# IDEA-Research/SegDINO3D

Hardware: AMD Instinct MI355X
Metric: scenes/sec forward (ScanNet200 ~150k pts, 200 queries) (higher is better)
Workload: dtype f32; 1 GPU; configs[1]: ScanNet-val-like scenes; a STEP is one scene; `value` times the K scenes as 28 evaluation forwards of 4/5 scenes each (`forward_sizes`), 4 forward(s) in flight per GPU (<= 20 scenes in flight); `single_scene` = one forward of one scene in flight; fp32 sparse backbone (Res16UNet34C) + fp32 decoder + post-processing, device-resident in/out; points=150000, superpoints=3000, queries_2d=300, scene_layout=benchmark, query_num=200, parallelism=scene-sharded x1, streams=4, max_scenes_per_forward=5, scenes_in_flight_per_gpu=20, gpu_numa_node=-1

## Files before the change

### include/segdino3d_hip.h

```cpp
#ifndef SEGDINO3D_HIP_H
#define SEGDINO3D_HIP_H

#include <stddef.h>
#include <stdint.h>

#ifdef __cplusplus
extern "C" {
#endif

#define SD3D_ABI_VERSION 2

int sd3d_abi_version(void);
const char* sd3d_last_error(void);
int sd3d_selftest_host(void);
int sd3d_set_scenes_in_flight(int n);

int sd3d_set_pair_pool(int on);
int sd3d_pair_pool_check(void);
int sd3d_pair_pool_launches(int64_t* launches_out);
int sd3d_pair_pool_poison(int64_t word);

size_t sd3d_sort_ws_bytes(int64_t n);
int sd3d_sort_pairs_u64_ex(uint64_t* keys_in, uint32_t* vals_in, uint64_t* keys_out, uint32_t* vals_out, uint32_t* vals_scratch,
                           int64_t n, int begin_bit, int end_bit, void* ws, size_t ws_bytes, int* landed_in_input, void* stream);
size_t sd3d_scan_ws_bytes(int64_t n);
int sd3d_scan_exclusive_i32(const int32_t* in, int32_t* out, int64_t n, int32_t* total_dev, void* ws, size_t ws_bytes,
                            void* stream);
int sd3d_keys_from_f32(const float* x, int64_t n, int descending, uint64_t* keys, void* stream);
int sd3d_keys_from_i64(const int64_t* x, int64_t n, uint64_t* keys, void* stream);
int sd3d_keys_from_i64_checked(const int64_t* x, int64_t n, uint64_t* keys, int bits, int32_t* flag, int flag_value, void* stream);
int sd3d_keys_from_i64_checked_max(const int64_t* x, int64_t n, uint64_t* keys, int bits, int32_t* flag, int flag_value, int32_t* max_out,
                                   void* stream);

int sd3d_keys_from_i64_offset_checked_max(const int64_t* x, int64_t n, int64_t add, uint64_t* keys, int bits, int32_t* flag, int flag_value,
                                          int32_t* max_out, void* stream);

size_t sd3d_scene_stats_ws_bytes(void);
int sd3d_scene_stats(const float* points, int ld, int64_t n, float* stats, void* ws, size_t ws_bytes, void* stream);
int sd3d_voxel_keys(const float* points, int ld, int64_t n, float inv_voxel, const float* stats, int shift_to_min,
                    int batch_index, int32_t* origin, uint64_t* keys, int32_t* icoords, int32_t* err_flag, void* stream);
size_t sd3d_unique_ws_bytes(int64_t n_cap);
int sd3d_unique_sorted(const uint64_t* keys, const uint32_t* src_idx, int64_t n_cap, const int32_t* n_dev, int shift,
                       uint64_t* ukeys, int32_t* seg_start, int32_t* map, int32_t* n_unique_dev, void* ws,
                       size_t ws_bytes, const float* clip_stats, float clip_inv_voxel, int clip_level, int clip_min_shape,
                       void* stream);
size_t sd3d_unique_levels_ws_bytes(int64_t n_cap, int n_extra);
int sd3d_unique_levels(const uint64_t* keys, int64_t n_cap, const int32_t* n_dev, int n_extra, uint64_t* const* ukeys,
                       int32_t* const* parents, int32_t* counts, void* ws, size_t ws_bytes, void* stream);
typedef struct sd3d_voxelise_desc {
    const float* points; int64_t n; int ld; int shift_to_min; float inv_voxel; int key_bits; int n_levels; int sp_bits;
// ... 375 lines not shown
```

### segdino3d_amd/_lib.py

```python
from __future__ import annotations

import ctypes as C
import os

_HERE = os.path.dirname(os.path.abspath(__file__))
LIB_PATH = os.environ.get("SD3D_LIB") or os.path.join(_HERE, "libsegdino3d_hip.so")
ABI_VERSION = 2

_lib = None

_p = C.c_void_p
_i = C.c_int
_l = C.c_int64
_z = C.c_size_t
_f = C.c_float

SIGNATURES = {
    "sd3d_abi_version": (_i, []),
    "sd3d_last_error": (C.c_char_p, []),
    "sd3d_set_scenes_in_flight": (_i, [_i]),
    "sd3d_set_pair_pool": (_i, [_i]),
    "sd3d_pair_pool_check": (_i, []),
    "sd3d_pair_pool_launches": (_i, [_p]),
    "sd3d_pair_pool_poison": (_i, [_l]),
    "sd3d_selftest_host": (_i, []),
    "sd3d_sort_ws_bytes": (_z, [_l]),
    "sd3d_sort_pairs_u64_ex": (_i, [_p, _p, _p, _p, _p, _l, _i, _i, _p, _z, _p, _p]),
    "sd3d_scan_ws_bytes": (_z, [_l]),
    "sd3d_scan_exclusive_i32": (_i, [_p, _p, _l, _p, _p, _z, _p]),
    "sd3d_keys_from_f32": (_i, [_p, _l, _i, _p, _p]),
    "sd3d_keys_from_i64": (_i, [_p, _l, _p, _p]),
    "sd3d_keys_from_i64_checked": (_i, [_p, _l, _p, _i, _p, _i, _p]),
    "sd3d_keys_from_i64_checked_max": (_i, [_p, _l, _p, _i, _p, _i, _p, _p]),
    "sd3d_keys_from_i64_offset_checked_max": (_i, [_p, _l, _l, _p, _i, _p, _i, _p, _p]),
    "sd3d_voxel_levels_all": (_i, [_p, _p, _l, _i, _p, _p, _p, _p, _p, _p, _z, _p]),
    "sd3d_voxelise_scene_ws_bytes": (_z, [_l, _i]),
    "sd3d_voxelise_scene": (_i, [_p, _p, _p]),
    "sd3d_scene_stats_ws_bytes": (_z, []),
    "sd3d_scene_stats": (_i, [_p, _i, _l, _p, _p, _z, _p]),
    "sd3d_voxel_keys": (_i, [_p, _i, _l, _f, _p, _i, _i, _p, _p, _p, _p, _p]),
    "sd3d_unique_ws_bytes": (_z, [_l]),
    "sd3d_unique_levels_ws_bytes": (_z, [_l, _i]),
    "sd3d_unique_levels": (_i, [_p, _l, _p, _i, _p, _p, _p, _p, _z, _p]),
    "sd3d_unique_sorted": (_i, [_p, _p, _l, _p, _i, _p, _p, _p, _p, _p, _z, _p, _f, _i, _i, _p]),
    "sd3d_hash_build": (_i, [_p, _l, _p, _p, _l, _p]),
    "sd3d_kernel_map": (_i, [_p, _l, _p, _p, _l, _p, _i, _i, _p, _p, _p]),
    "sd3d_kernel_maps_hier_ws_bytes": (_z, [_i, _p]),
    "sd3d_kernel_maps_hier": (_i, [_i, _p, _p, _p, _p, _p, _p, _p, _p, _p, _p, _p, _p, _p, _z, _p]),
    "sd3d_stride_maps": (_i, [_p, _p, _l, _l, _p, _p, _p, _p]),
    "sd3d_voxel_mean": (_i, [_p, _i, _p, _i, _i, _p, _l, _p, _p, _l, _p, _i, _p]),
    "sd3d_segment_starts": (_i, [_p, _l, _l, _p, _p]),
    "sd3d_voxel_mean_batch": (_i, [_p, _i, _i, _i, _p, _p, _p, _l, _p, _i, _p]),
    "sd3d_keys_from_i64_offset": (_i, [_p, _l, _l, _p, _p]),
    "sd3d_segment_starts_batch": (_i, [_p, _l, _l, _p, _i, _p, _p]),
# ... 140 lines not shown
```

### segdino3d_amd/csrc/pair_conv.h

```cpp
#pragma once
#include "common.h"
#include "../../include/segdino3d_hip.h"

#define PT 128
#define PG_CHAIN 0x40000000
#define PG_KMASK 0x3FFFFFFF

struct GGParams;

int launch_pair_conv(const float* in0, int ld0, int C0, const float* in1, int ld1, const int32_t* in_idx, const int32_t* tile_k,
                     int64_t p_cap, const int32_t* pos, const int32_t* rlist, int rl_stride, int center, const int32_t* out_idx,
                     const float* wt, int K, int Cin, int Cout, int64_t M, const float* scale,
                     const float* shift, const float* res, int ld_res, float* out, int ld_out, int act, float* part,
                     size_t part_bytes, hipStream_t st);
int launch_pair_dense(const GGParams& q, hipStream_t st);
```

### segdino3d_amd/csrc/pair_gemm.hip

```cpp
#include "gg_common.h"
#include "pair_conv.h"
#include <stdlib.h>
#include <atomic>
#include <vector>

static std::atomic<int> g_scenes_in_flight{1};
extern "C" int sd3d_set_scenes_in_flight(int n) { return g_scenes_in_flight.exchange(n < 1 ? 1 : n); }

#define PART_STORE4(PTR, V) do { if (p.nt_part) __builtin_nontemporal_store((V), (f32x4*)(PTR)); else *(f32x4*)(PTR) = (V); } while (0)
#define PART_LOAD4(PTR) __builtin_nontemporal_load((const f32x4*)(PTR))
#define PBS_LD 36

struct PGParams {
    const float* in0; int ld0; int C0;
    const float* in1; int ld1;
    const int32_t* in_idx;
    const int32_t* tile_k;
    const float* wt;
    int Cin, Cout;
    float* part;
    int n_tiles;
    const int32_t* out_idx;
    const float* scale; const float* shift; const float* res; int ld_res;
    float* out; int ld_out; int act;
// ... 15 lines not shown
    (void)__hip_atomic_fetch_max(ctr, (unsigned long long)epoch << 32, __ATOMIC_RELAXED, __HIP_MEMORY_SCOPE_AGENT);
}
__device__ __forceinline__ unsigned int pool_draw(unsigned long long* ctr, unsigned int epoch) {
    const unsigned long long old = __hip_atomic_fetch_add(ctr, 1ull, __ATOMIC_RELAXED, __HIP_MEMORY_SCOPE_AGENT);
    return (unsigned int)(old >> 32) == epoch ? (unsigned int)old : POOL_POISONED;
}
__global__ __launch_bounds__(256) void pool_check_kernel(unsigned long long tickets) {
    const int s = blockIdx.x * 256 + threadIdx.x;
    if (s >= PG_POOL_SLOTS) return;
    const unsigned long long last = tickets > (unsigned long long)s ? (tickets - 1 - s) / PG_POOL_SLOTS + 1 : 0;
    int bad = 0;
#pragma unroll
    for (int w = 0; w < PG_POOL_WORDS; ++w) {
        const unsigned long long v = g_pool_ctr[(size_t)s * PG_POOL_WORDS + w];
        if ((v >> 32) > last || ((v >> 32) == 0 && v != 0)) ++bad;
    }
    if (bad) atomicAdd(&g_pool_bad, (unsigned int)bad);
}


__device__ __forceinline__ float pg_affine(float x, const float* scale, const float* shift, int n) {
    return __builtin_fmaf(x, scale ? scale[n] : 1.f, shift ? shift[n] : 0.f);
}
__device__ __attribute__((noinline)) float pg_act_slow(float t, int act) {
    return act == 2 ? 0.5f * t * (1.f + erff(t * 0.70710678118654752440f)) : 1.f / (1.f + expf(-t));
}
__device__ __forceinline__ float pg_act(float t, int act) {
    if (act == 1) t = fmaxf(t, 0.f);
    else if (act >= 2) t = pg_act_slow(t, act);
    return t;
}

#define PG_PIECE 24
template <int NT, int MODE>
__device__ __forceinline__ void pair_gemm_body(const PGParams& p, float (*Bs)[NT * 32 * PBS_LD], int* Ix, int* Kx) {
    constexpr bool DIRECT = MODE >= 1;
    const int tid = threadIdx.x, lane = tid & 63;
    const int wv = __builtin_amdgcn_readfirstlane(tid >> 6);
    const int j = lane & 31, h = lane >> 5;
    constexpr bool dense = MODE == 2;
    const int n_real = dense ? (int)((p.dense_rows + PT - 1) / PT) : p.tile_k[p.n_tiles];
    const int nchunks = p.Cin >> 5;
    const bool pool = p.pool_ctr != nullptr && nchunks >= 3 && n_real >= 6 * (int)gridDim.x;
    int n_static = n_real;
    const int unit = (6 + nchunks - 1) / nchunks;
    if (pool) {
        if (tid == 0) pool_claim(p.pool_ctr + blockIdx.y, p.pool_epoch);
        n_static = (int)((int64_t)n_real * 13 / 16);
        if (p.chained) while (n_static < n_real && (p.tile_k[n_static - 1] & PG_CHAIN)) ++n_static;
    }
    int range0 = (int)((int64_t)blockIdx.x * n_static / gridDim.x);
    int range1 = (int)((int64_t)(blockIdx.x + 1) * n_static / gridDim.x);
    if (p.chained) {
        while (range0 > 0 && range0 < n_static && (p.tile_k[range0 - 1] & PG_CHAIN)) ++range0;
        while (range1 > 0 && range1 < n_static && (p.tile_k[range1 - 1] & PG_CHAIN)) ++range1;
    }
    if (range1 <= range0 && !pool) return;
    const int ncol0 = blockIdx.y * NT * 32;
    __shared__ int pool_unit;
    bool poisoned = false;
    int fallback_round = 0;
    const uint64_t wstride_b = (uint64_t)p.Cout * (uint64_t)p.Cin * 4ull;

    f32x16 acc[NT];
    const f32x16 zero16 = {0.f, 0.f, 0.f, 0.f, 0.f, 0.f, 0.f, 0.f, 0.f, 0.f, 0.f, 0.f, 0.f, 0.f, 0.f, 0.f};
    bool fresh = true;

    f32x4 bst[NT];
    uint32_t woff[NT];
#pragma unroll
    for (int i = 0; i < NT; ++i) {
        const int f = tid + i * 256;
        int n = ncol0 + (f >> 3);
        n = n < p.Cout ? n : p.Cout - 1;
        woff[i] = (uint32_t)(n * p.Cin + (f & 7) * 4) * 4u;
    }
    float* const sts = &Bs[0][(tid >> 3) * PBS_LD + (tid & 7) * 4];
    auto stage_load = [&](int kf, int chunk) {
        const int kw = p.k_flip >= 0 ? p.k_flip - (kf & PG_KMASK) : (kf & PG_KMASK);
        const char* Wk = (const char*)p.wt + (uint64_t)(uint32_t)kw * wstride_b + (uint32_t)chunk * 128u;
#pragma unroll
        for (int i = 0; i < NT; ++i) bst[i] = *(const f32x4*)(Wk + woff[i]);
    };
    auto stage_store = [&](int buf) {
#pragma unroll
        for (int i = 0; i < NT; ++i) *(f32x4*)(sts + buf * (NT * 32 * PBS_LD) + i * 32 * PBS_LD) = bst[i];
    };
    const uint64_t lane_b = (uint64_t)(h * 64);
    auto load_a = [&](f32x4 (&a)[4], int row, int chunk) {
        const int cc = chunk * 32;
        const bool first = cc < p.C0;
        const char* base = (const char*)(first ? p.in0 : p.in1) + (uint32_t)(first ? cc : cc - p.C0) * 4u;
        const uint32_t ld4 = (uint32_t)(first ? p.ld0 : p.ld1) * 4u;
        const char* src = base + ((uint64_t)(uint32_t)row * ld4 + lane_b);
#pragma unroll
        for (int q = 0; q < 4; ++q) a[q] = *(const f32x4*)(src + q * 16);
    };
    const bool full_cols = ncol0 + NT * 32 <= p.Cout;

  for (;;) {
    for (int piece0 = range0; piece0 < range1; piece0 += PG_PIECE) {
        const int ntl = range1 - piece0 < PG_PIECE ? range1 - piece0 : PG_PIECE;
        __syncthreads();
        if (dense) {
            for (int f = tid; f < ntl * PT; f += 256) {
                const int64_t r = (int64_t)piece0 * PT + f;
                Ix[f] = (int)(r < p.dense_rows ? r : p.dense_rows - 1);
            }
            if (tid < PG_PIECE + 2) Kx[tid] = 0;
        } else {
        for (int f = tid; f < ntl * PT; f += 256) {
            const int v = p.in_idx[(int64_t)piece0 * PT + f];
            Ix[f] = v < 0 ? 0 : v;
        }
        if (tid < PG_PIECE + 2) Kx[tid] = tid < ntl ? p.tile_k[piece0 + tid] : 0;
        }
        __syncthreads();
        const int nsteps = ntl * nchunks;
        const int* Iw = Ix + wv * 32 + j;
        int k_cur = __builtin_amdgcn_readfirstlane(Kx[0]), k_nxt = __builtin_amdgcn_readfirstlane(Kx[1]);
        f32x4 a0[4], a1[4], a2[4];
        int pf_t = 0, pf_c = 0;
#define PF_ADVANCE() do { if (++pf_c == nchunks) { pf_c = 0; ++pf_t; } } while (0)
#define PF_ROW() Iw[(pf_t < ntl ? pf_t : ntl - 1) * PT]
        load_a(a0, PF_ROW(), pf_c); PF_ADVANCE();
        load_a(a1, PF_ROW(), pf_c); PF_ADVANCE();
        stage_load(k_cur, 0);
        stage_store(0);
        __syncthreads();
        int buf = 0, cur_lt = 0, cur_c = 0, s = 0;
#define PAIR_STEP(CUR, PF)                                                                                            \
    {                                                                                                                 \
        const bool has_next = s + 1 < nsteps;                                                                         \
        const bool last_chunk = cur_c + 1 == nchunks;                                                                 \
        const int pf_row = PF_ROW();                 \
        const int k_after = Kx[cur_lt + 2];                                                                           \
        {                                                                                                             \
            const float* bb = &Bs[buf][j * PBS_LD + h * 16];                                                          \
            f32x4 bq[2][NT];                                                                                          \
            _Pragma("unroll") for (int t = 0; t < NT; ++t) bq[0][t] = *(const f32x4*)(bb + t * 32 * PBS_LD);          \
            _Pragma("unroll") for (int q = 0; q < 4; ++q) {                                                           \
                if (q < 3) {                                                                                          \
                    _Pragma("unroll") for (int t = 0; t < NT; ++t)                                                    \
                        bq[(q + 1) & 1][t] = *(const f32x4*)(bb + t * 32 * PBS_LD + (q + 1) * 4);                     \
                }                                                                                                     \
                _Pragma("unroll") for (int e = 0; e < 4; ++e) {                                                       \
                    if (q == 0 && e == 0) {                                                                           \
                        if (fresh) {                                                                                  \
// ... 37 lines not shown
                _Pragma("unroll") for (int t = 0; t < NT; ++t)                                                        \
                    _Pragma("unroll") for (int g = 0; g < 4; ++g)                                                     \
                        if (full_cols || ncol0 + 4 * h + t * 32 + 8 * g < p.Cout)                                     \
                            PART_STORE4(dst + t * 32 + 8 * g, (f32x4{acc[t][4 * g], acc[t][4 * g + 1],                \
                                                                     acc[t][4 * g + 2], acc[t][4 * g + 3]}));         \
            }                                                                                                         \
            fresh = true;                                                                                             \
        } else {                                                                                                      \
            fresh = false;                                                                                            \
        }                                                                                                             \
        if (!has_next) break;                                                                                         \
        stage_store(buf ^ 1);                                                                                         \
        __syncthreads();                                                                                              \
        buf ^= 1;                                                                                                     \
        ++s;                                                                                                          \
        if (last_chunk) {                                                                                             \
            cur_c = 0; ++cur_lt;                                                                                      \
            k_cur = k_nxt; k_nxt = __builtin_amdgcn_readfirstlane(k_after);                                           \
        } else {                                                                                                      \
            ++cur_c;                                                                                                  \
        }                                                                                                             \
    }
        for (;;) {
            PAIR_STEP(a0, a2)
            PAIR_STEP(a1, a0)
            PAIR_STEP(a2, a1)
        }
#undef PAIR_STEP
#undef PF_ADVANCE
#undef PF_ROW
    }
    if (!pool) break;
    __syncthreads();
    if (tid == 0) {
        unsigned int d = poisoned ? POOL_POISONED : pool_draw(p.pool_ctr + blockIdx.y, p.pool_epoch);
        if (d == POOL_POISONED) {
            if (!poisoned) atomicAdd(&g_pool_bad_seen, 1u);
            d = blockIdx.x + (unsigned)fallback_round * gridDim.x;
            pool_unit = -1 - (int)d;
        } else {
            pool_unit = (int)d;
        }
    }
    __syncthreads();
    int u = __builtin_amdgcn_readfirstlane(pool_unit);
    if (u < 0) { poisoned = true; ++fallback_round; u = -1 - u; }
    range0 = n_static + u * unit;
    if (range0 >= n_real) break;
    range1 = range0 + unit < n_real ? range0 + unit : n_real;
    if (p.chained) {
        while (range0 < n_real && (p.tile_k[range0 - 1] & PG_CHAIN)) ++range0;
        while (range1 < n_real && (p.tile_k[range1 - 1] & PG_CHAIN)) ++range1;
    }
  }
}

#define PAIR_GEMM_ENTRY(NAME, NT, WAVES, MODE)                                                                  \
    __global__ __launch_bounds__(256) __attribute__((amdgpu_waves_per_eu(WAVES, WAVES))) void NAME(const PGParams p) { \
        __shared__ __attribute__((aligned(16))) float Bs[2][NT * 32 * PBS_LD];                                  \
        __shared__ int Ix[PG_PIECE * PT];                                                                       \
        __shared__ int Kx[PG_PIECE + 2];                                                                        \
        pair_gemm_body<NT, MODE>(p, Bs, Ix, Kx);                                                               \
    }
PAIR_GEMM_ENTRY(pair_gemm_kernel_1, 1, 3, 0)
PAIR_GEMM_ENTRY(pair_gemm_kernel_2, 2, 2, 0)
PAIR_GEMM_ENTRY(pair_gemm_kernel_3, 3, 2, 0)
PAIR_GEMM_ENTRY(pair_gemm_kernel_4, 4, 2, 0)
PAIR_GEMM_ENTRY(pair_gemm_direct_kernel_1, 1, 3, 1)
PAIR_GEMM_ENTRY(pair_gemm_direct_kernel_2, 2, 2, 1)
PAIR_GEMM_ENTRY(pair_gemm_direct_kernel_3, 3, 2, 1)
PAIR_GEMM_ENTRY(pair_gemm_direct_kernel_4, 4, 2, 1)
PAIR_GEMM_ENTRY(pair_dense_kernel_1, 1, 3, 2)
PAIR_GEMM_ENTRY(pair_dense_kernel_2, 2, 2, 2)
PAIR_GEMM_ENTRY(pair_dense_kernel_3, 3, 2, 2)
PAIR_GEMM_ENTRY(pair_dense_kernel_4, 4, 2, 2)

#define WS_RANGE_TILES 24
#define WS_STAGE_BATCH 16

#define LOAD_A4(A, PTR)                                                                                            \
    do { _Pragma("unroll") for (int q_ = 0; q_ < 4; ++q_) A[q_] = *(const f32x4*)((PTR) + q_ * 4); } while (0)

template <int NT, int RT, int ST, bool DIRECT>
__device__ __forceinline__ void pair_gemm_ws_body(const PGParams& p, float* Ws) {
    constexpr int UPT = 4 / RT;
    const int tid = threadIdx.x, lane = tid & 63;
    const int wv = __builtin_amdgcn_readfirstlane(tid >> 6);
    const int j = lane & 31, h = lane >> 5;
    const int n_real = p.tile_k[p.n_tiles];
    const int range0 = (int)((int64_t)blockIdx.x * n_real / gridDim.x);
    const int range1 = (int)((int64_t)(blockIdx.x + 1) * n_real / gridDim.x);
    if (range1 <= range0) return;
    const int nchunks = p.Cin >> 5;
    const int ldw = p.Cin + 4;
    const int c4 = p.Cin >> 2;
    const int npieces = 32 * NT * c4;
    const int ncol0 = blockIdx.y * NT * 32;
    int* Ix = (int*)(Ws + 32 * NT * ldw);

    f32x16 acc[RT][NT];
    const f32x16 zero16 = {0.f, 0.f, 0.f, 0.f, 0.f, 0.f, 0.f, 0.f, 0.f, 0.f, 0.f, 0.f, 0.f, 0.f, 0.f, 0.f};
    bool fresh = true;

  for (int tile0 = range0; tile0 < range1; tile0 += WS_RANGE_TILES) {
    const int ntl = range1 - tile0 < WS_RANGE_TILES ? range1 - tile0 : WS_RANGE_TILES;
    __syncthreads();
    for (int f = tid; f < ntl * PT; f += 256) {
        const int v = p.in_idx[(int64_t)(tile0 + (f >> 7)) * PT + (f & (PT - 1))];
// ... 271 lines not shown
    if (hipDeviceSynchronize() != hipSuccess) { sd3d_set_error(SD3D_ERR_LAUNCH, "pair_pool_check: device synchronisation failed"); return -1; }
    unsigned int zero = 0, bad = 0, seen = 0;
    if (hipMemcpyToSymbol(HIP_SYMBOL(g_pool_bad), &zero, sizeof(zero)) != hipSuccess) { sd3d_set_error(SD3D_ERR_LAUNCH, "pair_pool_check: symbol write failed"); return -1; }
    hipLaunchKernelGGL(pool_check_kernel, dim3(PG_POOL_SLOTS / 256), dim3(256), 0, nullptr, g_pool_tickets[dev].load(std::memory_order_relaxed));
    if (hipGetLastError() != hipSuccess || hipDeviceSynchronize() != hipSuccess ||
        hipMemcpyFromSymbol(&bad, HIP_SYMBOL(g_pool_bad), sizeof(bad)) != hipSuccess ||
        hipMemcpyFromSymbol(&seen, HIP_SYMBOL(g_pool_bad_seen), sizeof(seen)) != hipSuccess ||
        hipMemcpyToSymbol(HIP_SYMBOL(g_pool_bad_seen), &zero, sizeof(zero)) != hipSuccess) { sd3d_set_error(SD3D_ERR_LAUNCH, "pair_pool_check: check kernel failed"); return -1; }
    if (seen) sd3d_set_error(SD3D_ERR_LAUNCH, "pair_pool_check: launches met counter words no launch can have written (they fell back to a static split of their shared tail: results unaffected)");
    bad += seen;
    return (int)bad;
}
extern "C" int sd3d_pair_pool_launches(int64_t* launches_out) {
    int dev = 0;
    if (!launches_out || hipGetDevice(&dev) != hipSuccess || dev < 0 || dev >= PG_MAX_DEVICES) return sd3d_set_error(SD3D_ERR_ARG, "pair_pool_launches: no device / no output");
    *launches_out = (int64_t)g_pool_tickets[dev].load(std::memory_order_relaxed);
    return SD3D_OK;
}
extern "C" int sd3d_pair_pool_poison(int64_t word) {
    unsigned long long* base = nullptr;
    if (hipGetSymbolAddress((void**)&base, HIP_SYMBOL(g_pool_ctr)) != hipSuccess) return sd3d_set_error(SD3D_ERR_LAUNCH, "pair_pool_poison: no symbol");
    std::vector<unsigned long long> h((size_t)PG_POOL_SLOTS * PG_POOL_WORDS, (unsigned long long)word);
    if (hipDeviceSynchronize() != hipSuccess || hipMemcpy(base, h.data(), h.size() * sizeof(unsigned long long), hipMemcpyHostToDevice) != hipSuccess)
        return sd3d_set_error(SD3D_ERR_LAUNCH, "pair_pool_poison: copy failed");
    return SD3D_OK;
}

typedef void (*PGKernel)(const PGParams);
static const PGKernel k_lockstep[2][4] = {{pair_gemm_kernel_1, pair_gemm_kernel_2, pair_gemm_kernel_3, pair_gemm_kernel_4},
                                          {pair_gemm_direct_kernel_1, pair_gemm_direct_kernel_2, pair_gemm_direct_kernel_3, pair_gemm_direct_kernel_4}};
static const PGKernel k_ws[2][4] = {{pair_gemm_ws_kernel_1, pair_gemm_ws_kernel_2, pair_gemm_ws_kernel_3, pair_gemm_ws_kernel_4},
                                    {pair_gemm_ws_direct_kernel_1, pair_gemm_ws_direct_kernel_2, pair_gemm_ws_direct_kernel_3, pair_gemm_ws_direct_kernel_4}};
static const PGKernel k_dense[4] = {pair_dense_kernel_1, pair_dense_kernel_2, pair_dense_kernel_3, pair_dense_kernel_4};

static std::atomic<int> g_n_cu[PG_MAX_DEVICES];
static std::atomic<bool> g_ws_attr[PG_MAX_DEVICES];

static int pg_device(int* n_cu) {
    int dev = 0;
    if (hipGetDevice(&dev) != hipSuccess || dev < 0 || dev >= PG_MAX_DEVICES) return -1;
    int n = g_n_cu[dev].load(std::memory_order_relaxed);
    if (!n) {
        if (hipDeviceGetAttribute(&n, hipDeviceAttributeMultiprocessorCount, dev) != hipSuccess || n <= 0) return -1;
        g_n_cu[dev].store(n, std::memory_order_relaxed);
    }
    *n_cu = n;
    return dev;
}

static void pg_col_tiles(int Cout, int* nt_out, int* cgs_out) {
    const int sub = (Cout + 31) / 32;
    int nt = sub >= 4 ? 4 : sub;
    if (sub > 4 && sub % 4) { for (int c = 4; c >= 1; --c) if (sub % c == 0) { nt = c; break; } }
    *nt_out = nt;
    *cgs_out = (int)cdiv(sub, nt);
}

static dim3 pg_lockstep_grid(int n_cu, int nt, int cgs, int64_t tiles) {
    int gx = n_cu * (nt == 1 ? 3 : 2) / cgs;
    gx = gx < 1 ? 1 : (gx < tiles ? gx : (int)tiles);
    return dim3((unsigned)gx, (unsigned)cgs);
}

static void pg_setup_pool(PGParams& g, int dev, int cgs, hipStream_t st) {
    if (!pool_enabled() || cgs > PG_POOL_WORDS) return;
    hipStreamCaptureStatus cap = hipStreamCaptureStatusNone;
    if (st != nullptr && (hipStreamIsCapturing(st, &cap) != hipSuccess || cap != hipStreamCaptureStatusNone)) return;
    unsigned long long* base = g_pool_bases[dev].load(std::memory_order_acquire);
    if (!base && hipGetSymbolAddress((void**)&base, HIP_SYMBOL(g_pool_ctr)) == hipSuccess) g_pool_bases[dev].store(base, std::memory_order_release);
    if (!base) return;
    const unsigned long long t = g_pool_tickets[dev].fetch_add(1, std::memory_order_relaxed);
    g.pool_ctr = base + (size_t)(t % PG_POOL_SLOTS) * PG_POOL_WORDS;
    g.pool_epoch = (unsigned int)(t / PG_POOL_SLOTS + 1);
}

int launch_pair_conv(const float* in0, int ld0, int C0, const float* in1, int ld1, const int32_t* in_idx, const int32_t* tile_k,
                     int64_t p_cap, const int32_t* pos, const int32_t* rlist, int rl_stride, int center, const int32_t* out_idx,
                     const float* wt, int K, int Cin, int Cout, int64_t M, const float* scale,
                     const float* shift, const float* res, int ld_res, float* out, int ld_out, int act, float* part,
                     size_t part_bytes, hipStream_t st) {
    if (M <= 0 || Cout <= 0) return SD3D_OK;
    if (Cin <= 0 || (Cin & 31)) return sd3d_set_error(SD3D_ERR_ARG, "pair_conv: Cin must be a positive multiple of 32");
    if (Cout & 3) return sd3d_set_error(SD3D_ERR_ARG, "pair_conv: Cout must be a multiple of 4");
    if (in1 && ((C0 & 31) || C0 > Cin)) return sd3d_set_error(SD3D_ERR_ARG, "pair_conv: concat split must be a multiple of 32");
    if (!in1) C0 = Cin;
    if ((ld0 & 3) || (in1 && (ld1 & 3)) || (ld_out & 3)) return sd3d_set_error(SD3D_ERR_ARG, "pair_conv: row strides must be multiples of 4 floats");
    if (p_cap <= 0 || (p_cap % PT)) return sd3d_set_error(SD3D_ERR_ARG, "pair_conv: p_cap must be a positive multiple of 128");
    if (part_bytes < (size_t)p_cap * Cout * sizeof(float)) return sd3d_set_error(SD3D_ERR_ARG, "pair_conv: partial-product buffer too small");
    int n_cu = 0;
    const int dev = pg_device(&n_cu);
    if (dev < 0) return sd3d_set_error(SD3D_ERR_LAUNCH, "pair_conv: no device");
    if ((ld_res & 3) && res) return sd3d_set_error(SD3D_ERR_ARG, "pair_conv: residual row stride must be a multiple of 4 floats");
    const bool mirror_w = center == SD3D_PAIR_MIRROR_W(-1) || center == SD3D_PAIR_MIRROR_W(SD3D_PAIR_CHAINED);
    if (mirror_w) center += 2;
    if (center >= 0 || center < SD3D_PAIR_CHAINED) return sd3d_set_error(SD3D_ERR_ARG, "pair_conv: center must be -1 or SD3D_PAIR_CHAINED, or SD3D_PAIR_MIRROR_W of them (the dense centre kernel of round 3 left the library: profiles/EXPERIMENTS.md)");
    const bool direct = out_idx != nullptr;
    if (!direct && !rlist && !pos)
        return sd3d_set_error(SD3D_ERR_ARG, "pair_conv: pass 2 needs rlist, or pos, or out_idx (direct epilogue); "
                                            "this table was built without a position table (lean evaluation lists)");
    const bool crowded = g_scenes_in_flight.load(std::memory_order_relaxed) > 1;
    PGParams g;
    g.in0 = in0; g.ld0 = ld0; g.C0 = C0; g.in1 = in1; g.ld1 = ld1; g.in_idx = in_idx; g.tile_k = tile_k; g.wt = wt;
    g.Cin = Cin; g.Cout = Cout; g.part = part;
    g.chained = center == SD3D_PAIR_CHAINED ? 1 : 0;
    g.nt_part = crowded ? 1 : 0;
    g.dense_rows = 0;
    g.pool_ctr = nullptr;
    g.pool_epoch = 0;
    g.k_flip = mirror_w ? K - 1 : -1;
    g.out_idx = out_idx;
    g.scale = scale; g.shift = shift; g.res = res; g.ld_res = ld_res; g.out = out; g.ld_out = ld_out; g.act = act;
    int nt, cgs;
    pg_col_tiles(Cout, &nt, &cgs);
    g.n_tiles = (int)(p_cap / PT);
    const size_t w_lds = (size_t)Cout * (Cin + 4) * sizeof(float);
    const size_t w_lds_cg = (size_t)(32 * nt) * (Cin + 4) * sizeof(float);
    const bool ws_one = !g.chained && !(crowded && nt >= 3) && cgs == 1 && Cout == 32 * nt && w_lds <= 68 * 1024;
    const bool ws_two = !g.chained && !crowded && cgs == 2 && nt == 4 && Cout == 256 && g.n_tiles >= 1024 && w_lds_cg + WS_RANGE_TILES * PT * sizeof(int32_t) + 256 <= 160 * 1024;
    if (ws_one || ws_two) {
        if (!g_ws_attr[dev].load(std::memory_order_relaxed)) {
            for (int d = 0; d < 2; ++d)
                for (int i = 0; i < 4; ++i)
                    (void)hipFuncSetAttribute((const void*)k_ws[d][i], hipFuncAttributeMaxDynamicSharedMemorySize, (i == 3 ? 160 : 80) * 1024);
            g_ws_attr[dev].store(true, std::memory_order_relaxed);
        }
        int per_cu = nt == 1 ? 4 : (nt == 3 ? 3 : 2);
        const size_t w_need = ws_two ? w_lds_cg : w_lds;
        const int by_lds = (int)((160 * 1024) / (w_need + WS_RANGE_TILES * PT * sizeof(int32_t) + 256));
        per_cu = per_cu < by_lds ? per_cu : by_lds;
        int gx = n_cu * per_cu / (ws_two ? 2 : 1);
        gx = gx < 1 ? 1 : (gx < g.n_tiles ? gx : g.n_tiles);
        const size_t lds = w_need + (size_t)WS_RANGE_TILES * PT * sizeof(int32_t);
        hipLaunchKernelGGL(k_ws[direct][nt - 1], dim3((unsigned)gx, ws_two ? 2u : 1u), dim3(256), lds, st, g);
    } else {
        pg_setup_pool(g, dev, cgs, st);
        hipLaunchKernelGGL(k_lockstep[direct][nt - 1], pg_lockstep_grid(n_cu, nt, cgs, g.n_tiles), dim3(256), 0, st, g);
    }
    if (direct) {
    } else if (rlist) {
        PRLParams r;
        r.rlist = rlist; r.rl_stride = rl_stride; r.M = M; r.part = part; r.Cout = Cout; r.scale = scale; r.shift = shift; r.res = res;
        r.ld_res = ld_res; r.out = out; r.ld_out = ld_out; r.act = act;
        hipLaunchKernelGGL(pair_reduce_rl_kernel, dim3((unsigned)cdiv(M * (Cout / 4), 256)), dim3(256), 0, st, r);
    } else {
        PRParams r;
        r.pos = pos; r.K = K; r.M = M; r.part = part; r.Cout = Cout; r.scale = scale; r.shift = shift; r.res = res; r.ld_res = ld_res;
        r.out = out; r.ld_out = ld_out; r.act = act;
        hipLaunchKernelGGL(pair_reduce_kernel, dim3((unsigned)cdiv(M * (Cout / 4), 256)), dim3(256), 0, st, r);
    }
    SD3D_CHECK_LAUNCH();
    return SD3D_OK;
}
extern "C" int sd3d_pair_conv_ex(const float* in0, int ld0, int C0, const float* in1, int ld1, const int32_t* in_idx, const int32_t* tile_k,
                                 int64_t p_cap, const int32_t* pos, const int32_t* rlist, int rl_stride, int center, const int32_t* out_idx,
                                 const float* wt, int K, int Cin, int Cout, int64_t M, const float* scale, const float* shift, const float* res,
                                 int ld_res, float* out, int ld_out, int act, float* part, size_t part_bytes, void* stream) {
    return launch_pair_conv(in0, ld0, C0, in1, ld1, in_idx, tile_k, p_cap, pos, rlist, rl_stride, center, out_idx, wt, K, Cin, Cout, M,
                            scale, shift, res, ld_res, out, ld_out, act, part, part_bytes, (hipStream_t)stream);
}

int launch_pair_dense(const GGParams& q, hipStream_t st) {
    int n_cu = 0;
    if (pg_device(&n_cu) < 0) return sd3d_set_error(SD3D_ERR_LAUNCH, "pair_dense: no device");
    PGParams g;
    g.in0 = q.in0; g.ld0 = q.ld0; g.C0 = q.in1 ? q.C0 : q.Cin; g.in1 = q.in1; g.ld1 = q.ld1; g.in_idx = nullptr; g.tile_k = nullptr; g.wt = q.wt;
    g.Cin = q.Cin; g.Cout = q.Cout; g.part = nullptr; g.n_tiles = 0; g.out_idx = nullptr; g.scale = q.scale; g.shift = q.shift; g.res = q.res;
    g.ld_res = q.ld_res; g.out = q.out; g.ld_out = q.ld_out; g.act = q.act; g.nt_part = 0; g.chained = 0; g.dense_rows = q.M; g.pool_ctr = nullptr; g.pool_epoch = 0; g.k_flip = -1;
    int nt, cgs;
    pg_col_tiles(q.Cout, &nt, &cgs);
// ... 5 lines not shown
```

### segdino3d_amd/csrc/pair_lists.hip

```cpp
#include "pair_conv.h"

#define PL_ROWS 2048

__device__ static inline int block_excl_scan_256p(int v, int* total, int* smem4) {
    const int lane = threadIdx.x & 63, w = threadIdx.x >> 6;
    int inc = v;
#pragma unroll
    for (int d = 1; d < 64; d <<= 1) {
        int t = __shfl_up(inc, d);
        if (lane >= d) inc += t;
    }
    if (lane == 63) smem4[w] = inc;
    __syncthreads();
    int base = 0;
    for (int i = 0; i < w; ++i) base += smem4[i];
    *total = smem4[0] + smem4[1] + smem4[2] + smem4[3];
    __syncthreads();
    return base + inc - v;
}

#define PL_MAX_TABLES 16
#define RL_ROWS 256
struct PLTable {
    const int32_t* nbr; int32_t* pos; int32_t* in_idx; int32_t* tile_k; int32_t* blk_cnt; int32_t* totals;
// ... 356 lines not shown
    __syncthreads();
    for (int sg = tid; sg < nseg; sg += 256) {
        int run = T.blk_cnt[(int64_t)sg * T.nblk + blk];
#pragma unroll
        for (int w = 0; w < 4; ++w) { const int c = wb[w][sg]; wb[w][sg] = run; run += c; }
    }
    __syncthreads();
    for (int sg = blk; sg < nseg; sg += T.nblk) {
        const int g = sg / CH_NPAT, q = sg - g * CH_NPAT;
        const int ns = g == T.G ? 1 : ch_nsrc(q), nt = (seg_tot[sg] + PT - 1) / PT;
        for (int e = tid; e < nt * ns; e += 256) {
            const int sub = e % ns;
            int k;
            if (g == T.G) k = centre;
            else if (q == 0) k = g;
            else if (q == 1) k = T.K - 1 - g;
            else if (q == 2) k = sub == 0 ? g : T.K - 1 - g;
            else if (q == 3) k = sub == 0 ? centre : g;
            else if (q == 4) k = sub == 0 ? centre : T.K - 1 - g;
            else k = sub == 0 ? centre : (sub == 1 ? g : T.K - 1 - g);
            if ((int64_t)(seg_tile[sg] + e) * PT < T.p_cap) T.tile_k[seg_tile[sg] + e] = k | (sub < ns - 1 ? PG_CHAIN : 0);
        }
        if (nt > 0) {
            const int fill0 = seg_tot[sg] - (nt - 1) * PT;
            for (int e = tid; e < (PT - fill0) * ns; e += 256) {
                const int sub = e / (PT - fill0), off = fill0 + e % (PT - fill0);
                const int64_t pp = (int64_t)(seg_tile[sg] + (nt - 1) * ns + sub) * PT + off;
                if (pp < T.p_cap) T.in_idx[pp] = -1;
            }
        }
    }
    {
        const int64_t cap_tiles = T.p_cap / PT;
        if (blk == 0 && tid == 0) { T.tile_k[cap_tiles] = (int)(end_tile < cap_tiles ? end_tile : cap_tiles); T.tile_k[cap_tiles + 1] = 0; T.tile_k[cap_tiles + 2] = 0; }
        if (!T.lean) {
            for (int64_t e = (int64_t)end_tile * PT + (int64_t)blk * 256 + tid; e < T.p_cap; e += (int64_t)T.nblk * 256) T.in_idx[e] = -1;
            for (int64_t tt = end_tile + (int64_t)blk * 256 + tid; tt < cap_tiles; tt += (int64_t)T.nblk * 256) T.tile_k[tt] = -1;
        }
    }
    const uint64_t lt = (1ull << lane) - 1ull;
    int32_t* rl = T.rlist + (live ? row : 0) * T.rl_stride;
    int cnt = 0;
    ch_walk(T, row, live, [&](int g, int pat, int ia, int ib) {
        uint64_t mine = 0;
#pragma unroll
        for (int q = 0; q < CH_NPAT; ++q) {
            const uint64_t bal = __ballot(pat == q);
            if (pat == q) mine = bal;
        }
        if (pat >= 0) {
            const int sg = g * CH_NPAT + pat, ns = ch_nsrc(pat);
            const int my = wb[wv][sg] + __popcll(mine & lt);
            const int64_t tile = seg_tile[sg] + (int64_t)(my >> 7) * ns;
            const int off = my & (PT - 1);
            if ((tile + ns) * PT <= T.p_cap) {
                int64_t pp = tile * PT + off;
                if (pat >= 3) { T.in_idx[pp] = (int)row; pp += PT; }
                if (ia >= 0) { T.in_idx[pp] = ia; pp += PT; }
                if (ib >= 0) { T.in_idx[pp] = ib; pp += PT; }
                rl[1 + cnt++] = (int32_t)(pp - PT);
            }
        }
    });
    {
        const bool lone = live && !any;
        const uint64_t bal = __ballot(lone);
        if (lone) {
// ... 129 lines not shown
```

### segdino3d_amd/sparse.py

```python
from __future__ import annotations

from typing import Sequence, Dict, Optional, Tuple

import os

import numpy as np
import torch

from . import ops

_OFFSET_CACHE: Dict[Tuple[int, str, str], torch.Tensor] = {}


def kernel_offsets_np(ksize: int, order: str) -> np.ndarray:
    r = np.arange(ksize) - (ksize - 1) // 2 if ksize % 2 else np.arange(ksize)
    if order == "x_fastest":
        z, y, x = np.meshgrid(r, r, r, indexing="ij")
    elif order == "z_fastest":
        x, y, z = np.meshgrid(r, r, r, indexing="ij")
    else:
        raise ValueError(order)
    return np.stack([x.ravel(), y.ravel(), z.ravel()], axis=1).astype(np.int8)


# ... 31 lines not shown


def _device_memory(device) -> int:
    idx = torch.cuda.current_device() if device is None or device.index is None else device.index
    if idx not in _TOTAL_MEM:
        _TOTAL_MEM[idx] = int(torch.cuda.get_device_properties(idx).total_memory)
    return _TOTAL_MEM[idx]


def exact_pair_capacity(n_vox0: int, device=None) -> bool:
    if EXACT_PAIR_CAPACITY == "auto":
        return (ops.scenes_in_flight_now() > 1 or n_vox0 > WORST_CASE_MAX_VOXELS
                or 125 * 32 * 4 * n_vox0 > WORST_CASE_MEM_FRACTION * _device_memory(device))
    return bool(EXACT_PAIR_CAPACITY)


HIER_MAPS = os.environ.get("SD3D_HIER_MAPS", "1") != "0"
_INV27 = {}


def inv27_table(order: str) -> np.ndarray:
    if order not in _INV27:
        offs = kernel_offsets_np(3, order).astype(np.int64)
        inv = np.zeros(27, dtype=np.int8)
        for k, (dx, dy, dz) in enumerate(offs):
            inv[(dx + 1) + 3 * (dy + 1) + 9 * (dz + 1)] = k
        _INV27[order] = inv
    return _INV27[order]


MIRRORED_MAPS = os.environ.get("SD3D_MIRRORED_MAPS", "1") != "0"

PAIR_CHAIN = os.environ.get("SD3D_PAIR_CHAIN", "1") != "0"
PAIR_CHAIN_LEVELS = tuple(int(v) for v in os.environ.get("SD3D_PAIR_CHAIN_LEVELS", "0,1,2").split(",") if v.strip() != "")
FORK_JOIN = os.environ.get("SD3D_FORK_JOIN", "0") != "0"
OPTIMISTIC_SORT = os.environ.get("SD3D_OPTIMISTIC_SORT", "1") != "0"
LEVELS_AT_ONCE = os.environ.get("SD3D_LEVELS_AT_ONCE", "1") != "0"
LEAN_LISTS = os.environ.get("SD3D_LEAN_LISTS", "1") != "0"
VOXELISE_ONE_CALL = os.environ.get("SD3D_VOXELISE_ONE_CALL", "1") != "0"
MORTON_BITS = 48


def _levels_at_once(n_levels: int, clip_min_shape: int) -> bool:
    return LEVELS_AT_ONCE and clip_min_shape == 0 and 1 < n_levels <= 8


def _levels_from_sorted(skeys, sidx, n_levels: int, rb, clip=None):
    N = skeys.shape[0]
    at_once = _levels_at_once(n_levels, clip[2] if clip else 0)
    if at_once and VOXELISE_ONE_CALL:
        return ops.voxel_levels_all(skeys, sidx, n_levels, rb[0:n_levels])
    ukeys, seg_start, inverse, n_prev = ops.unique_sorted(
        skeys, sidx, N, None, 0, want_seg_start=True, want_map=True, map_size=N, nuniq_out=rb[0:1])
    if at_once:
        uks, parents, _ = ops.unique_levels(ukeys, N, n_prev, n_levels - 1, counts_out=rb[1:n_levels])
        return [ukeys] + uks, seg_start, inverse, parents
    keys_l, parents = [ukeys], []
    for lvl in range(1, n_levels):
        uk, _, parent, n_prev = ops.unique_sorted(keys_l[-1], None, N, n_prev, 3, want_seg_start=False, want_map=True,
                                                  clip=(clip[0], clip[1], lvl, clip[2]) if clip else None, nuniq_out=rb[lvl:lvl + 1])
        keys_l.append(uk)
        parents.append(parent)
    return keys_l, seg_start, inverse, parents


class SceneMaps:

# ... 350 lines not shown
```

Before: 125.6 scenes/s.

## Add wide 512-thread pair-GEMM kernel, balanced chain cuts, and chain level 3

Adds a 512-thread pair-GEMM variant in which two 256-thread groups each cover one half of the 256 output columns, sharing the gathered index tiles in LDS. The variant is gated behind SD3D_PAIR_WIDE and is off by default. Chain-boundary handling now snaps each cut to the nearer chain end using PG_MAX_CHAIN instead of always walking forward, and the tile_k count is clamped to whole chains when capacity overflows. Chaining is also enabled by default for sparse level 3. That extends the gather-sharing chained path to another level, at some risk of worse load balance.

```diff
diff --git a/include/segdino3d_hip.h b/include/segdino3d_hip.h
--- a/include/segdino3d_hip.h
+++ b/include/segdino3d_hip.h
@@ -16,6 +16,7 @@
 int sd3d_set_scenes_in_flight(int n);
 
 int sd3d_set_pair_pool(int on);
+int sd3d_set_pair_launch(int grid_x, int wide);
 int sd3d_pair_pool_check(void);
 int sd3d_pair_pool_launches(int64_t* launches_out);
 int sd3d_pair_pool_poison(int64_t word);
diff --git a/segdino3d_amd/_lib.py b/segdino3d_amd/_lib.py
--- a/segdino3d_amd/_lib.py
+++ b/segdino3d_amd/_lib.py
@@ -20,6 +20,7 @@
     "sd3d_last_error": (C.c_char_p, []),
     "sd3d_set_scenes_in_flight": (_i, [_i]),
     "sd3d_set_pair_pool": (_i, [_i]),
+    "sd3d_set_pair_launch": (_i, [_i, _i]),
     "sd3d_pair_pool_check": (_i, []),
     "sd3d_pair_pool_launches": (_i, [_p]),
     "sd3d_pair_pool_poison": (_i, [_l]),
diff --git a/segdino3d_amd/csrc/pair_conv.h b/segdino3d_amd/csrc/pair_conv.h
--- a/segdino3d_amd/csrc/pair_conv.h
+++ b/segdino3d_amd/csrc/pair_conv.h
@@ -5,6 +5,7 @@
 #define PT 128
 #define PG_CHAIN 0x40000000
 #define PG_KMASK 0x3FFFFFFF
+#define PG_MAX_CHAIN 3
 
 struct GGParams;
 
diff --git a/segdino3d_amd/csrc/pair_gemm.hip b/segdino3d_amd/csrc/pair_gemm.hip
--- a/segdino3d_amd/csrc/pair_gemm.hip
+++ b/segdino3d_amd/csrc/pair_gemm.hip
@@ -71,31 +71,48 @@
 }
 
 #define PG_PIECE 24
-template <int NT, int MODE>
+__device__ __forceinline__ int pg_chain_cut(const int32_t* tile_k, int b, int n) {
+    static_assert(PG_MAX_CHAIN == 3, "pg_chain_cut reads the flags of tiles b - 2 ... b");
+    if (b <= 0) return 0;
+    if (b >= n) return n;
+    if (!(tile_k[b - 1] & PG_CHAIN)) return b;
+    const int s = (b >= 2 && (tile_k[b - 2] & PG_CHAIN)) ? b - 2 : b - 1;
+    int e = (tile_k[b] & PG_CHAIN) ? b + 2 : b + 1;
+    e = e < n ? e : n;
+    return e - b < b - s ? e : s;
+}
+
+template <int NT, int MODE, int GROUPS>
 __device__ __forceinline__ void pair_gemm_body(const PGParams& p, float (*Bs)[NT * 32 * PBS_LD], int* Ix, int* Kx) {
     constexpr bool DIRECT = MODE >= 1;
-    const int tid = threadIdx.x, lane = tid & 63;
+    constexpr int NTHR = 256 * GROUPS;
+    const int tid_wg = threadIdx.x;
+    const int tid = tid_wg & 255, lane = tid & 63;
     const int wv = __builtin_amdgcn_readfirstlane(tid >> 6);
+    const int grp = GROUPS > 1 ? __builtin_amdgcn_readfirstlane(tid_wg >> 8) : 0;
+    const int pool_word = GROUPS > 1 ? 0 : (int)blockIdx.y;
+    Bs += 2 * grp;
     const int j = lane & 31, h = lane >> 5;
     constexpr bool dense = MODE == 2;
     const int n_real = dense ? (int)((p.dense_rows + PT - 1) / PT) : p.tile_k[p.n_tiles];
     const int nchunks = p.Cin >> 5;
     const bool pool = p.pool_ctr != nullptr && nchunks >= 3 && n_real >= 6 * (int)gridDim.x;
     int n_static = n_real;
-    const int unit = (6 + nchunks - 1) / nchunks;
+    int unit = (6 + nchunks - 1) / nchunks;
+    if (p.chained && unit < PG_MAX_CHAIN) unit = PG_MAX_CHAIN;
     if (pool) {
-        if (tid == 0) pool_claim(p.pool_ctr + blockIdx.y, p.pool_epoch);
+        if (tid_wg == 0) pool_claim(p.pool_ctr + pool_word, p.pool_epoch);
         n_static = (int)((int64_t)n_real * 13 / 16);
-        if (p.chained) while (n_static < n_real && (p.tile_k[n_static - 1] & PG_CHAIN)) ++n_static;
+        if (p.chained) n_static = pg_chain_cut(p.tile_k, n_static, n_real);
     }
     int range0 = (int)((int64_t)blockIdx.x * n_static / gridDim.x);
     int range1 = (int)((int64_t)(blockIdx.x + 1) * n_static / gridDim.x);
     if (p.chained) {
-        while (range0 > 0 && range0 < n_static && (p.tile_k[range0 - 1] & PG_CHAIN)) ++range0;
-        while (range1 > 0 && range1 < n_static && (p.tile_k[range1 - 1] & PG_CHAIN)) ++range1;
+        range0 = pg_chain_cut(p.tile_k, range0, n_static);
+        range1 = pg_chain_cut(p.tile_k, range1, n_static);
     }
     if (range1 <= range0 && !pool) return;
-    const int ncol0 = blockIdx.y * NT * 32;
+    const int ncol0 = (GROUPS > 1 ? grp : (int)blockIdx.y) * NT * 32;
     __shared__ int pool_unit;
     bool poisoned = false;
     int fallback_round = 0;
@@ -142,17 +159,17 @@
         const int ntl = range1 - piece0 < PG_PIECE ? range1 - piece0 : PG_PIECE;
         __syncthreads();
         if (dense) {
-            for (int f = tid; f < ntl * PT; f += 256) {
+            for (int f = tid_wg; f < ntl * PT; f += NTHR) {
                 const int64_t r = (int64_t)piece0 * PT + f;
                 Ix[f] = (int)(r < p.dense_rows ? r : p.dense_rows - 1);
             }
-            if (tid < PG_PIECE + 2) Kx[tid] = 0;
+            if (tid_wg < PG_PIECE + 2) Kx[tid_wg] = 0;
         } else {
-        for (int f = tid; f < ntl * PT; f += 256) {
+        for (int f = tid_wg; f < ntl * PT; f += NTHR) {
             const int v = p.in_idx[(int64_t)piece0 * PT + f];
             Ix[f] = v < 0 ? 0 : v;
         }
-        if (tid < PG_PIECE + 2) Kx[tid] = tid < ntl ? p.tile_k[piece0 + tid] : 0;
+        if (tid_wg < PG_PIECE + 2) Kx[tid_wg] = tid_wg < ntl ? p.tile_k[piece0 + tid_wg] : 0;
         }
         __syncthreads();
         const int nsteps = ntl * nchunks;
@@ -256,8 +273,8 @@
     }
     if (!pool) break;
     __syncthreads();
-    if (tid == 0) {
-        unsigned int d = poisoned ? POOL_POISONED : pool_draw(p.pool_ctr + blockIdx.y, p.pool_epoch);
+    if (tid_wg == 0) {
+        unsigned int d = poisoned ? POOL_POISONED : pool_draw(p.pool_ctr + pool_word, p.pool_epoch);
         if (d == POOL_POISONED) {
             if (!poisoned) atomicAdd(&g_pool_bad_seen, 1u);
             d = blockIdx.x + (unsigned)fallback_round * gridDim.x;
@@ -273,8 +290,8 @@
     if (range0 >= n_real) break;
     range1 = range0 + unit < n_real ? range0 + unit : n_real;
     if (p.chained) {
-        while (range0 < n_real && (p.tile_k[range0 - 1] & PG_CHAIN)) ++range0;
-        while (range1 < n_real && (p.tile_k[range1 - 1] & PG_CHAIN)) ++range1;
+        range0 = pg_chain_cut(p.tile_k, range0, n_real);
+        range1 = pg_chain_cut(p.tile_k, range1, n_real);
     }
   }
 }
@@ -284,7 +301,7 @@
         __shared__ __attribute__((aligned(16))) float Bs[2][NT * 32 * PBS_LD];                                  \
         __shared__ int Ix[PG_PIECE * PT];                                                                       \
         __shared__ int Kx[PG_PIECE + 2];                                                                        \
-        pair_gemm_body<NT, MODE>(p, Bs, Ix, Kx);                                                               \
+        pair_gemm_body<NT, MODE, 1>(p, Bs, Ix, Kx);                                                            \
     }
 PAIR_GEMM_ENTRY(pair_gemm_kernel_1, 1, 3, 0)
 PAIR_GEMM_ENTRY(pair_gemm_kernel_2, 2, 2, 0)
@@ -298,6 +315,16 @@
 PAIR_GEMM_ENTRY(pair_dense_kernel_2, 2, 2, 2)
 PAIR_GEMM_ENTRY(pair_dense_kernel_3, 3, 2, 2)
 PAIR_GEMM_ENTRY(pair_dense_kernel_4, 4, 2, 2)
+#define PG_WIDE_LDS (size_t)(4 * 4 * 32 * PBS_LD * sizeof(float) + PG_PIECE * PT * sizeof(int) + (PG_PIECE + 2) * sizeof(int))
+#define PAIR_GEMM_WIDE_ENTRY(NAME, MODE)                                                                        \
+    __global__ __launch_bounds__(512) __attribute__((amdgpu_waves_per_eu(2, 2))) void NAME(const PGParams p) {  \
+        extern __shared__ __attribute__((aligned(16))) float wide_smem[];                                       \
+        float (*Bs)[4 * 32 * PBS_LD] = (float (*)[4 * 32 * PBS_LD])wide_smem;                                   \
+        int* Ix = (int*)(wide_smem + 4 * 4 * 32 * PBS_LD);                                                      \
+        pair_gemm_body<4, MODE, 2>(p, Bs, Ix, Ix + PG_PIECE * PT);                                             \
+    }
+PAIR_GEMM_WIDE_ENTRY(pair_gemm_wide_kernel, 0)
+PAIR_GEMM_WIDE_ENTRY(pair_gemm_wide_direct_kernel, 1)
 
 #define WS_RANGE_TILES 24
 #define WS_STAGE_BATCH 16
@@ -635,9 +662,29 @@
 static const PGKernel k_ws[2][4] = {{pair_gemm_ws_kernel_1, pair_gemm_ws_kernel_2, pair_gemm_ws_kernel_3, pair_gemm_ws_kernel_4},
                                     {pair_gemm_ws_direct_kernel_1, pair_gemm_ws_direct_kernel_2, pair_gemm_ws_direct_kernel_3, pair_gemm_ws_direct_kernel_4}};
 static const PGKernel k_dense[4] = {pair_dense_kernel_1, pair_dense_kernel_2, pair_dense_kernel_3, pair_dense_kernel_4};
+static const PGKernel k_wide[2] = {pair_gemm_wide_kernel, pair_gemm_wide_direct_kernel};
 
 static std::atomic<int> g_n_cu[PG_MAX_DEVICES];
 static std::atomic<bool> g_ws_attr[PG_MAX_DEVICES];
+static std::atomic<bool> g_wide_attr[PG_MAX_DEVICES];
+static std::atomic<int> g_grid_cap{0};
+static std::atomic<int> g_wide_sw{-2};
+static int pair_wide_switch() {
+    int v = g_wide_sw.load(std::memory_order_relaxed);
+    if (v == -2) {
+        const char* e = getenv("SD3D_PAIR_WIDE");
+        int expected = -2;
+        g_wide_sw.compare_exchange_strong(expected, e && *e ? (atoi(e) != 0) : -1);
+        v = g_wide_sw.load(std::memory_order_relaxed);
+    }
+    return v;
+}
+extern "C" int sd3d_set_pair_launch(int grid_x, int wide) {
+    (void)pair_wide_switch();
+    g_grid_cap.store(grid_x > 0 ? grid_x : 0, std::memory_order_relaxed);
+    g_wide_sw.store(wide < 0 ? -1 : (wide != 0), std::memory_order_relaxed);
+    return SD3D_OK;
+}
 
 static int pg_device(int* n_cu) {
     int dev = 0;
@@ -659,8 +706,9 @@
     *cgs_out = (int)cdiv(sub, nt);
 }
 
-static dim3 pg_lockstep_grid(int n_cu, int nt, int cgs, int64_t tiles) {
+static dim3 pg_lockstep_grid(int n_cu, int nt, int cgs, int64_t tiles, int cap = 0) {
     int gx = n_cu * (nt == 1 ? 3 : 2) / cgs;
+    if (cap > 0 && cap < gx) gx = cap;
     gx = gx < 1 ? 1 : (gx < tiles ? gx : (int)tiles);
     return dim3((unsigned)gx, (unsigned)cgs);
 }
@@ -720,6 +768,9 @@
     const size_t w_lds_cg = (size_t)(32 * nt) * (Cin + 4) * sizeof(float);
     const bool ws_one = !g.chained && !(crowded && nt >= 3) && cgs == 1 && Cout == 32 * nt && w_lds <= 68 * 1024;
     const bool ws_two = !g.chained && !crowded && cgs == 2 && nt == 4 && Cout == 256 && g.n_tiles >= 1024 && w_lds_cg + WS_RANGE_TILES * PT * sizeof(int32_t) + 256 <= 160 * 1024;
+    const int wide_sw = pair_wide_switch();
+    const int grid_cap = g_grid_cap.load(std::memory_order_relaxed);
+    const bool wide = !ws_one && !ws_two && cgs == 2 && nt == 4 && Cout == 256 && wide_sw > 0;
     if (ws_one || ws_two) {
         if (!g_ws_attr[dev].load(std::memory_order_relaxed)) {
             for (int d = 0; d < 2; ++d)
@@ -735,9 +786,16 @@
         gx = gx < 1 ? 1 : (gx < g.n_tiles ? gx : g.n_tiles);
         const size_t lds = w_need + (size_t)WS_RANGE_TILES * PT * sizeof(int32_t);
         hipLaunchKernelGGL(k_ws[direct][nt - 1], dim3((unsigned)gx, ws_two ? 2u : 1u), dim3(256), lds, st, g);
+    } else if (wide) {
+        if (!g_wide_attr[dev].load(std::memory_order_relaxed)) {
+            for (int d = 0; d < 2; ++d) (void)hipFuncSetAttribute((const void*)k_wide[d], hipFuncAttributeMaxDynamicSharedMemorySize, (int)PG_WIDE_LDS);
+            g_wide_attr[dev].store(true, std::memory_order_relaxed);
+        }
+        pg_setup_pool(g, dev, 1, st);
+        hipLaunchKernelGGL(k_wide[direct], dim3(pg_lockstep_grid(n_cu, nt, cgs, g.n_tiles, grid_cap).x), dim3(512), PG_WIDE_LDS, st, g);
     } else {
         pg_setup_pool(g, dev, cgs, st);
-        hipLaunchKernelGGL(k_lockstep[direct][nt - 1], pg_lockstep_grid(n_cu, nt, cgs, g.n_tiles), dim3(256), 0, st, g);
+        hipLaunchKernelGGL(k_lockstep[direct][nt - 1], pg_lockstep_grid(n_cu, nt, cgs, g.n_tiles, grid_cap), dim3(256), 0, st, g);
     }
     if (direct) {
     } else if (rlist) {
diff --git a/segdino3d_amd/csrc/pair_lists.hip b/segdino3d_amd/csrc/pair_lists.hip
--- a/segdino3d_amd/csrc/pair_lists.hip
+++ b/segdino3d_amd/csrc/pair_lists.hip
@@ -412,7 +412,20 @@
     }
     {
         const int64_t cap_tiles = T.p_cap / PT;
-        if (blk == 0 && tid == 0) { T.tile_k[cap_tiles] = (int)(end_tile < cap_tiles ? end_tile : cap_tiles); T.tile_k[cap_tiles + 1] = 0; T.tile_k[cap_tiles + 2] = 0; }
+        if (blk == 0 && tid == 0) {
+            int64_t n_real = end_tile;
+            if (end_tile > cap_tiles) {
+                n_real = 0;
+                for (int sg = 0; sg < nseg; ++sg) {
+                    const int ns = sg == nseg - 1 ? 1 : ch_nsrc(sg % CH_NPAT);
+                    const int64_t first = seg_tile[sg], tiles = (int64_t)(seg_tot[sg] + PT - 1) / PT * ns;
+                    if (first + tiles <= cap_tiles) { n_real = first + tiles; continue; }
+                    if (first < cap_tiles) n_real = first + (cap_tiles - first) / ns * ns;
+                    break;
+                }
+            }
+            T.tile_k[cap_tiles] = (int)n_real; T.tile_k[cap_tiles + 1] = 0; T.tile_k[cap_tiles + 2] = 0;
+        }
         if (!T.lean) {
             for (int64_t e = (int64_t)end_tile * PT + (int64_t)blk * 256 + tid; e < T.p_cap; e += (int64_t)T.nblk * 256) T.in_idx[e] = -1;
             for (int64_t tt = end_tile + (int64_t)blk * 256 + tid; tt < cap_tiles; tt += (int64_t)T.nblk * 256) T.tile_k[tt] = -1;
diff --git a/segdino3d_amd/sparse.py b/segdino3d_amd/sparse.py
--- a/segdino3d_amd/sparse.py
+++ b/segdino3d_amd/sparse.py
@@ -87,7 +87,7 @@
 MIRRORED_MAPS = os.environ.get("SD3D_MIRRORED_MAPS", "1") != "0"
 
 PAIR_CHAIN = os.environ.get("SD3D_PAIR_CHAIN", "1") != "0"
-PAIR_CHAIN_LEVELS = tuple(int(v) for v in os.environ.get("SD3D_PAIR_CHAIN_LEVELS", "0,1,2").split(",") if v.strip() != "")
+PAIR_CHAIN_LEVELS = tuple(int(v) for v in os.environ.get("SD3D_PAIR_CHAIN_LEVELS", "0,1,2,3").split(",") if v.strip() != "")
 FORK_JOIN = os.environ.get("SD3D_FORK_JOIN", "0") != "0"
 OPTIMISTIC_SORT = os.environ.get("SD3D_OPTIMISTIC_SORT", "1") != "0"
 LEVELS_AT_ONCE = os.environ.get("SD3D_LEVELS_AT_ONCE", "1") != "0"
```

Result: faster. 128.4 scenes/s, median of 6 (+2.2%).
